# Thealexbarney/VGAudio

Hardware: AMD Instinct MI355X
Metric: Msamples/s encoded (GC-ADPCM, 4096 ch) at 1/2/4/8 GPUs; % HBM roofline (higher is better)
Workload: dtype int32; 1 GPU; BASELINE configs[1]: 4096 mono channels x 48 kHz x 60 s GC-ADPCM coefficient search + encode per GPU; parallelism=units sharded x1, channels_per_gpu=4096, samples_per_channel=2880000, bit_exact_channels_checked=0

## Files before the change

include/vgaudio_hip_testing.h:

```cpp
#ifndef VGAUDIO_HIP_TESTING_H
#define VGAUDIO_HIP_TESTING_H

#ifdef __cplusplus
extern "C" {
#endif

int vga_testing_force_open_seams_this_thread(int mode);

int vga_testing_gc_encoder_layout_this_thread(int channels_per_wave);
int vga_testing_gc_coefs_variant_this_thread(int variant);
int vga_testing_gc_encoder_segments_this_thread(int segments);
int vga_testing_gc_encoder_persistent_this_thread(int mode);

int vga_testing_gc_plan_pieces(int cus, int groups, int frames, long long group_frames, int ragged, int *out5);
int vga_testing_gc_plan_pieces_n(int cus, int groups, int frames, long long group_frames, int ragged, int coarse, int *out10);

int vga_testing_gc_encode_stats(unsigned long long *out8, int reset);
int vga_testing_gc_encode_stats_n(unsigned long long *out, int n, int reset);

int vga_testing_gc_seam_handover_this_thread(int on);
int vga_testing_gc_schedule_this_thread(int big_rounds, const int *tail_counts, const int *tail_frames, int min_tail_frames);
int vga_testing_gc_slow_order_host(const short *coefs, int nch, int *order);
int vga_testing_gc_slow_order_device(const void *d_coefs, int nch, int *order);
int vga_testing_gc_prologue_device(const void *d_coefs, int nch, int zero_ints, int *order_flags, int *bad_words);

void vga_testing_host_pipeline_this_thread(int feeders, int drainers, int chunk_units, int slot_bytes);

void vga_testing_host_pipeline_tail_this_thread(int tail_units);

int vga_testing_plan_buckets(const int *group, const int *length, int n, int max_units, long long max_volume, int longest_first,
                             int *order_out, int *chunk_begin_out, int *chunk_length_out, int *chunk_group_out, int max_chunks);
void vga_testing_buckets_order_this_thread(int order);
void vga_testing_host_transfer_this_thread(int mode);
void vga_testing_host_transfer_piece_bytes_this_thread(int bytes);
void vga_testing_host_compute_lanes_this_thread(int lanes);

enum {
    VGA_TESTING_STEP_CHUNK_COMPUTE = 1,
    VGA_TESTING_STEP_TRANSFER = 2,
    VGA_TESTING_STEP_HCA_STREAM_FRAMES = 3
};
void vga_testing_fail_step_this_thread(int kind, int nth);

int vga_testing_last_pipeline_stats(double *out, int n);

int vga_testing_hca_frames_per_group_this_thread(int frames);

int vga_testing_hca_device_info(const void *hca_info, void *out, int out_bytes);

int vga_testing_hca_decode_classes(const void *infos, int nstreams, int *class_out);
int vga_testing_hca_decode_v_stats(long long *out, int n);
int vga_testing_hca_ragged_stats(const void *ragged, long long *out, int n);

int vga_testing_adx_read_general_this_thread(int on);

int vga_testing_adx_last_path_this_thread(int *encode, int *decode);
int vga_testing_adx_ragged_stats(const void *ragged, long long *out, int n);

int vga_testing_poison_allocations(int byte);

#ifdef __cplusplus
}
#endif
// ... 2 lines not shown
```

vgaudio_amd/_lib.py:

```python
import ctypes as C
import importlib.util
import os

_HERE = os.path.dirname(os.path.abspath(__file__))
SO_PATH = os.environ.get("VGAUDIO_HIP_LIBRARY") or os.path.join(_HERE, "libvgaudio_hip.so")

VGA_OK = 0
VGA_ERR_ARGUMENT = -1
VGA_ERR_OUT_OF_RANGE = -2
VGA_ERR_INVALID_DATA = -3
VGA_ERR_INVALID_OP = -4
VGA_ERR_DEVICE = -5

VGA_TESTING_STEP_CHUNK_COMPUTE = 1
VGA_TESTING_STEP_TRANSFER = 2
VGA_TESTING_STEP_HCA_STREAM_FRAMES = 3


class VgaError(RuntimeError):
    code = None


class ArgumentError(VgaError, ValueError):
    code = VGA_ERR_ARGUMENT
# ... 80 lines not shown
    "vga_gcadpcm_encode_with_coefs_batch_v": (ci, [i16pp, C.POINTER(ci), ci, i16p, i16p, i16p, u8pp]),
    "vga_gcadpcm_decode_batch_v": (ci, [u8pp, i16p, C.POINTER(ci), ci, i16p, i16p, i16pp]),
    "vga_gcadpcm_ragged_create": (ci, [C.POINTER(ci), ci, C.POINTER(vp)]),
    "vga_gcadpcm_ragged_destroy": (None, [vp]),
    "vga_gcadpcm_ragged_channels": (ci, [vp]),
    "vga_gcadpcm_ragged_pcm_samples": (i64, [vp]),
    "vga_gcadpcm_ragged_adpcm_bytes": (i64, [vp]),
    "vga_gcadpcm_ragged_coefs_workspace_bytes": (C.c_size_t, [vp]),
    "vga_gcadpcm_ragged_offsets": (ci, [vp, C.POINTER(i64), C.POINTER(i64)]),
    "vga_gcadpcm_coefs_device_v": (ci, [vp, vp, vp, vp, C.c_size_t, vp]),
    "vga_gcadpcm_encode_device_v": (ci, [vp, vp, vp, vp, vp, vp, vp]),
    "vga_gcadpcm_decode_device_v": (ci, [vp, vp, vp, vp, vp, vp, vp, vp]),
    "encode": (None, [i16p, u8p, C.POINTER(ADPCMINFO), C.c_uint32]),
    "decode": (None, [u8p, i16p, C.POINTER(ADPCMINFO), C.c_uint32]),
    "correlateCoefs": (None, [i16p, C.c_uint32, i16p]),
    "encodeFrame": (None, [i16p, u8p, i16p, C.c_uint8]),
    "vga_gcadpcm_coefs_workspace_bytes": (C.c_size_t, [ci, ci]),
    "vga_gcadpcm_coefs_device": (ci, [vp, i64, ci, ci, vp, vp, C.c_size_t, vp]),
    "vga_gcadpcm_encode_device": (ci, [vp, i64, ci, ci, vp, vp, vp, vp, i64, vp]),
    "vga_gcadpcm_decode_device": (ci, [vp, i64, vp, ci, ci, vp, vp, vp, i64, vp, vp]),
    "vga_synth_pcm16_device": (ci, [vp, i64, ci, ci, ci, vp, vp]),
    "vga_adx_file_layout_for": (ci, [vp, ci, vp]),
    "vga_adx_write": (ci, [u8pp, ci, i16p, ci, vp, u8p]),
    "vga_adx_write_device": (ci, [vp, i64, ci, vp, ci, vp, vp, vp]),
    "vga_hca_file_size": (ci, [vp]),
    "vga_hca_file_header": (ci, [vp, C.c_char_p, C.c_float, ci, ci, u8p]),
    "vga_hca_write": (ci, [vp, u8p, C.c_char_p, C.c_float, ci, ci, u8p]),
    "vga_hca_write_device": (ci, [vp, vp, i64, ci, C.c_char_p, C.c_float, ci, ci, vp, i64, vp]),
    "vga_wave_parse": (ci, [u8p, i64, vp]),
    "vga_wave_read_pcm16": (ci, [u8p, i64, vp, i16pp]),
    "vga_wave_deinterleave_pcm16_device": (ci, [vp, ci, ci, vp, i64, vp]),
    "vga_wave_file_size": (i64, [vp, ci]),
    "vga_wave_write_pcm16": (ci, [i16pp, ci, vp, u8p]),
    "vga_wave_write_pcm16_device": (ci, [vp, i64, ci, vp, vp, vp]),
    "vga_adx_key_from_code": (ci, [C.c_uint64, vp]),
    "vga_adx_key_from_string": (ci, [C.c_char_p, vp]),
    "vga_adx_key_code": (C.c_uint64, [vp]),
    "vga_adx_crypt": (ci, [u8pp, ci, ci, vp, ci, ci]),
    "vga_adx_crypt_device": (ci, [vp, i64, ci, ci, vp, ci, ci, vp]),
    "vga_adx_find_key_device": (ci, [vp, i64, ci, ci, ci, ci, vp, ci, C.POINTER(ci), vp]),
    "vga_hca_key_tables": (ci, [ci, C.c_uint64, u8p, u8p]),
    "vga_hca_crypt": (ci, [u8p, ci, ci, u8p]),
    "vga_hca_find_key": (ci, [vp, u8p, ci, u8p, ci, vp]),
    "vga_hca_find_key_device": (ci, [vp, vp, ci, u8p, ci, vp, vp]),
    "vga_hca_byte_position_counts_device": (ci, [vp, i64, ci, ci, ci, ci, vp, vp]),
    "vga_adx_guess_default_candidates": (ci, [ci, vp, vp, vp, vp]),
    "vga_adx_guess_keys": (ci, [vp, ci, ci, ci, vp, ci, vp, ci, vp, ci, vp]),
    "vga_hca_crypt_device": (ci, [vp, i64, ci, ci, ci, u8p, vp]),
    "vga_release_cached_memory": (None, []),
    "vga_testing_force_open_seams_this_thread": (ci, [ci]),
    "vga_testing_host_pipeline_this_thread": (None, [ci, ci, ci, ci]),
    "vga_testing_gc_encoder_layout_this_thread": (ci, [ci]),
    "vga_testing_gc_coefs_variant_this_thread": (ci, [ci]),
    "vga_testing_gc_encoder_segments_this_thread": (ci, [ci]),
    "vga_testing_gc_encoder_persistent_this_thread": (ci, [ci]),
    "vga_testing_gc_seam_handover_this_thread": (ci, [ci]),
    "vga_testing_gc_schedule_this_thread": (ci, [ci, C.POINTER(ci), C.POINTER(ci), ci]),
    "vga_testing_gc_slow_order_host": (ci, [vp, ci, vp]),
    "vga_testing_gc_slow_order_device": (ci, [vp, ci, vp]),
    "vga_testing_gc_prologue_device": (ci, [vp, ci, ci, vp, vp]),
    "vga_testing_gc_encode_stats_n": (ci, [C.POINTER(C.c_ulonglong), ci, ci]),
    "vga_testing_last_pipeline_stats": (ci, [vp, ci]),
    "vga_testing_host_pipeline_tail_this_thread": (None, [ci]),
    "vga_testing_buckets_order_this_thread": (None, [ci]),
    "vga_testing_host_transfer_this_thread": (None, [ci]),
    "vga_testing_host_transfer_piece_bytes_this_thread": (None, [ci]),
    "vga_testing_host_compute_lanes_this_thread": (None, [ci]),
    "vga_testing_fail_step_this_thread": (None, [ci, ci]),
    "vga_testing_poison_allocations": (ci, [ci]),
    "vga_testing_plan_buckets": (ci, [C.POINTER(ci), C.POINTER(ci), ci, ci, C.c_longlong, ci, C.POINTER(ci), C.POINTER(ci), C.POINTER(ci),
                                 C.POINTER(ci), ci]),
    "vga_testing_hca_device_info": (ci, [vp, vp, ci]),
    "vga_testing_hca_decode_classes": (ci, [vp, ci, C.POINTER(ci)]),
    "vga_testing_hca_decode_v_stats": (ci, [C.POINTER(C.c_longlong), ci]),
    "vga_testing_hca_ragged_stats": (ci, [vp, C.POINTER(C.c_longlong), ci]),
    "vga_hca_ragged_layout_for": (ci, [vp, ci, C.POINTER(i64), C.POINTER(i64), vp]),
    "vga_hca_ragged_create": (ci, [vp, ci, C.POINTER(vp)]),
    "vga_hca_ragged_destroy": (None, [vp]),
    "vga_hca_ragged_streams": (ci, [vp]),
    "vga_hca_ragged_totals_of": (ci, [vp, vp]),
    "vga_hca_ragged_offsets": (ci, [vp, C.POINTER(i64), C.POINTER(i64)]),
    "vga_testing_adx_ragged_stats": (ci, [vp, C.POINTER(C.c_longlong), ci]),
    "vga_adx_ragged_layout_for": (ci, [vp, C.POINTER(ci), ci, C.POINTER(i64), C.POINTER(i64), vp]),
    "vga_adx_ragged_create": (ci, [vp, C.POINTER(ci), ci, C.POINTER(vp)]),
    "vga_adx_ragged_destroy": (None, [vp]),
    "vga_adx_ragged_channels": (ci, [vp]),
    "vga_adx_ragged_totals_of": (ci, [vp, vp]),
    "vga_adx_ragged_offsets": (ci, [vp, C.POINTER(i64), C.POINTER(i64)]),
    "vga_adx_encode_device_v": (ci, [vp, vp, vp, vp, vp, C.c_size_t, vp]),
    "vga_adx_decode_device_v": (ci, [vp, vp, vp, vp, C.c_size_t, vp, vp]),
    "vga_gc_files_layout_for": (ci, [vp, ci, vp, C.POINTER(ci), C.POINTER(i64), C.POINTER(i64), vp]),
    "vga_gc_files_create": (ci, [vp, ci, vp, C.POINTER(vp)]),
    "vga_gc_files_create_from_dsp": (ci, [C.POINTER(vp), ci, C.POINTER(i64), C.POINTER(vp)]),
    "vga_gc_files_destroy": (None, [vp]),
    "vga_gc_files_totals_of": (ci, [vp, vp]),
    "vga_gc_files_offsets": (ci, [vp, C.POINTER(ci), C.POINTER(i64), C.POINTER(i64)]),
    "vga_gc_files_ragged": (vp, [vp]),
    "vga_gcadpcm_build_channels_device_v": (ci, [vp, vp, vp, vp, vp, vp, vp, vp, C.c_size_t, vp]),
    "vga_dsp_write_device_v": (ci, [vp, vp, vp, vp, vp, vp, vp, vp]),
    "vga_dsp_read_device_v": (ci, [vp, vp, vp, vp, vp, vp, vp, vp]),
    "vga_gc_aligned_layout_for": (ci, [vp, ci, C.POINTER(ci), C.POINTER(i64), vp]),
    "vga_gc_aligned_create": (ci, [vp, ci, C.POINTER(vp)]),
    "vga_gc_aligned_destroy": (None, [vp]),
    "vga_gc_aligned_totals_of": (ci, [vp, vp]),
    "vga_gc_aligned_offsets": (ci, [vp, C.POINTER(ci), C.POINTER(i64)]),
    "vga_gc_aligned_ragged_in": (vp, [vp]),
# ... 564 lines not shown
```

vgaudio_amd/csrc/gcadpcm_kernels.hip:

```cpp
#include "common.hpp"
#include "gcadpcm_kernels.hpp"

#include <algorithm>
#include <cstdlib>
#include <type_traits>

namespace vga {
namespace gc {

struct Record {
    double r1, r2;
    bool valid;
};

__device__ __forceinline__ double get3(const double (&v)[3], int i) { return i == 0 ? v[0] : (i == 1 ? v[1] : v[2]); }
__device__ __forceinline__ void set3(double (&v)[3], int i, double val)
{
    if (i == 0) v[0] = val; else if (i == 1) v[1] = val; else v[2] = val;
}

struct FrameSums {
    double vec[3];
    double m11, m12, m22;
};

__device__ __forceinline__ FrameSums frame_sums(const int (&x)[16])
{
    FrameSums f;
#pragma unroll
    for (int i = 0; i <= 2; i++) {
        long long s = 0;
#pragma unroll
        for (int t = 0; t < 14; t++) s -= (long long)(x[2 + t - i] * x[2 + t]);
        f.vec[i] = (double)s;
    }
    long long s11 = 0, s12 = 0, s22 = 0;
#pragma unroll
    for (int z = 0; z < 14; z++) {
        s11 += (long long)(x[2 + z - 1] * x[2 + z - 1]);
        s12 += (long long)(x[2 + z - 1] * x[2 + z - 2]);
        s22 += (long long)(x[2 + z - 2] * x[2 + z - 2]);
    }
    f.m11 = (double)s11; f.m12 = (double)s12; f.m22 = (double)s22;
    return f;
}

typedef short short2v __attribute__((ext_vector_type(2)));
__device__ __forceinline__ int dot2_less1(uint32_t a, uint32_t b)
{
    return __builtin_amdgcn_sdot2(__builtin_bit_cast(short2v, a), __builtin_bit_cast(short2v, b), -1, false);
}
__device__ __forceinline__ FrameSums frame_sums_packed(const uint32_t (&w)[8])
{
    double s0 = 7.0, s1 = 7.0, s2 = 7.0;
#pragma unroll
    for (int i = 0; i < 7; i++) {
        s0 += (double)dot2_less1(w[i + 1], w[i + 1]);
        s1 += (double)dot2_less1(w[i], __builtin_amdgcn_alignbit(w[i + 1], w[i], 16));
        s2 += (double)dot2_less1(w[i], w[i + 1]);
    }
    const int x0 = (int)(int16_t)(w[0] & 0xFFFF), x1 = (int)w[0] >> 16;
    const int x14 = (int)(int16_t)(w[7] & 0xFFFF), x15 = (int)w[7] >> 16;
    FrameSums f;
    f.vec[0] = 0.0 - s0;
    f.vec[1] = 0.0 - ((s1 - (double)(x0 * x1)) + (double)(x14 * x15));
    f.vec[2] = 0.0 - s2;
    f.m12 = s1;
    f.m11 = (s0 + (double)(x1 * x1)) - (double)(x15 * x15);
    f.m22 = (f.m11 + (double)(x0 * x0)) - (double)(x14 * x14);
    return f;
}

__device__ __forceinline__ Record frame_record(const FrameSums &fs)
{
    Record rec;
    rec.valid = false;
    rec.r1 = rec.r2 = 0.0;

    double vec[3] = {fs.vec[0], fs.vec[1], fs.vec[2]};
    if (!(fabs(vec[0]) > 10.0)) return rec;

    double m11 = fs.m11, m12 = fs.m12, m21 = fs.m12, m22 = fs.m22;

    int idx1, idx2;
    {
        const double eps = 4.9406564584124654e-324;
        double val = fmax(fabs(m11), fabs(m12));
        if (val < eps) return rec;
        double rc1 = 1.0 / val;
        val = fmax(fabs(m21), fabs(m22));
        if (val < eps) return rec;
        double rc2 = 1.0 / val;

        int max_index = 0;
        double tmp;
        val = 0.0;
        tmp = fabs(m11) * rc1;
        if (tmp >= val) { val = tmp; max_index = 1; }
        tmp = fabs(m21) * rc2;
        if (tmp >= val) { val = tmp; max_index = 2; }
        if (max_index == 2) {
            double t;
            t = m21; m21 = m11; m11 = t;
            t = m22; m22 = m12; m12 = t;
            rc2 = rc1;
        }
        idx1 = max_index;
        tmp = 1.0 / m11;
        m21 *= tmp;
        val = 0.0;
        tmp = m22;
        tmp -= m21 * m12;
        m22 = tmp;
        tmp = fabs(tmp) * rc2;
        if (tmp >= val) { val = tmp; max_index = 2; }
        if (max_index == 1) {
            double t;
            t = m11; m11 = m21; m21 = t;
            t = m12; m12 = m22; m22 = t;
            rc1 = rc2;
        }
        idx2 = max_index;

        double mn = 1.0e10, mx = 0.0;
        tmp = fabs(m11);
        if (tmp < mn) mn = tmp;
        if (tmp > mx) mx = tmp;
        tmp = fabs(m22);
        if (tmp < mn) mn = tmp;
        if (tmp > mx) mx = tmp;
        if (mn / mx < 1.0e-10) return rec;
    }

    {
        double tmp;
        int xx = 0;
        tmp = get3(vec, idx1);
        set3(vec, idx1, vec[1]);
        if (xx != 0) {  }
        else if (tmp != 0.0) xx = 1;
        vec[1] = tmp;
        tmp = get3(vec, idx2);
        set3(vec, idx2, vec[2]);
        if (xx != 0) {
            if (xx == 1) tmp -= vec[1] * m21;
        } else if (tmp != 0.0) xx = 2;
        vec[2] = tmp;

        tmp = vec[2];
        vec[2] = tmp / m22;
        tmp = vec[1];
        tmp -= vec[2] * m12;
        vec[1] = tmp / m11;
        vec[0] = 1.0;
    }

    {
        const double v2 = vec[2];
        const double tmp = 1.0 - (v2 * v2);
        if (tmp == 0.0) return rec;
        const double v0 = (vec[0] - (v2 * v2)) / tmp;
        const double v1 = (vec[1] - (vec[1] * v2)) / tmp;
        vec[0] = v0;
        vec[1] = v1;
        if (fabs(v1) > 1.0) return rec;
    }

#pragma unroll
    for (int z = 1; z <= 2; z++) {
        if (vec[z] >= 1.0) vec[z] = 0.9999999999;
        else if (vec[z] <= -1.0) vec[z] = -0.9999999999;
    }
    rec.r1 = (vec[2] * vec[1]) + vec[1];
    rec.r2 = vec[2];
    rec.valid = true;
    return rec;
}

__device__ __forceinline__ void matrix_filter(double r1, double r2, double &d1, double &d2)
{
    const double m21 = -r1;
    const double m22 = -r2;
    const double val = 1.0 - (m22 * m22);
    const double m11 = ((m22 * m21) + m21) / val;
    d1 = 0.0 + m11 * 1.0;
    d2 = (0.0 + m21 * d1) + m22 * 1.0;
}

__device__ __forceinline__ void finish_record(double (&in_r)[3], double (&out_r)[3])
{
#pragma unroll
    for (int z = 1; z <= 2; z++) {
        if (in_r[z] >= 1.0) in_r[z] = 0.9999999999;
        else if (in_r[z] <= -1.0) in_r[z] = -0.9999999999;
    }
    out_r[0] = 1.0;
    out_r[1] = (in_r[2] * in_r[1]) + in_r[1];
    out_r[2] = in_r[2];
}

__device__ void merge_finish_record(const double (&src)[3], double (&dst)[3])
{
    double tmp[3] = {0.0, 0.0, 0.0};
    double val = src[0];
    dst[0] = 1.0;
    {
        double v2 = 0.0;
        if (val > 0.0) dst[1] = -(v2 + src[1]) / val;
        else dst[1] = 0.0;
        tmp[1] = dst[1];
        val *= 1.0 - (dst[1] * dst[1]);
    }
    {
        double v2 = 0.0;
        v2 += dst[1] * src[1];
        if (val > 0.0) dst[2] = -(v2 + src[2]) / val;
        else dst[2] = 0.0;
        tmp[2] = dst[2];
        dst[1] += dst[2] * dst[1];
        val *= 1.0 - (dst[2] * dst[2]);
    }
    finish_record(tmp, dst);
}


__device__ __forceinline__ void load_frame16(const int16_t *src, int f, int length, int (&x)[16])
{
    const int base = f * 14 - 2;
    if (f > 0 && base + 16 <= length) {
        const uint32_t *p32 = reinterpret_cast<const uint32_t *>(src + base);
#pragma unroll
        for (int i = 0; i < 8; i++) {
            const uint32_t w = p32[i];
            x[2 * i] = (int)(int16_t)(w & 0xFFFF);
            x[2 * i + 1] = (int)w >> 16;
        }
    } else {
#pragma unroll
        for (int i = 0; i < 16; i++) {
// ... 104 lines not shown
    __shared__ double s_vb[8][3];
    __shared__ double s_cw[8][3];
    __shared__ double s_sum[8][3];
    __shared__ int s_cnt[8];

    const int ch = rg.order ? rg.order[blockIdx.x] : (int)blockIdx.x;
    if (rg.order) length = rg.length[ch];
    const int lane = threadIdx.x;
    const int16_t *src = pcm + (rg.order ? rg.pcm_off[ch] : (int64_t)ch * pcm_pitch);
    const int frames = (length + 13) / 14;
    const int rec_pitch = (int)coef_record_pitch(frames);
    double2 *rec = records + (rg.order ? rg.rec_off[ch] : (int64_t)ch * rec_pitch);
    const int my_bucket = lane >> 1;
    const int my_comp = lane & 1;
    uint32_t wave_slot = 0;
    if (VGA_COEFS_PRIO == 1) asm volatile("s_getreg_b32 %0, hwreg(HW_REG_HW_ID, 0, 4)" : "=s"(wave_slot));
    if (VGA_COEFS_PRIO == 3) __builtin_amdgcn_s_setprio(3);
    const int64_t ragged_job = rg.order ? (int64_t)((rg.max_length + 13) / 14) * 7 : 0;
    auto ragged_priority = [&](int passes_left) __attribute__((always_inline)) {
        const int64_t q = 4 * (int64_t)frames * passes_left / (ragged_job > 0 ? ragged_job : 1);
        set_priority((uint32_t)(q > 3 ? 3 : q));
    };
    if (VGA_COEFS_PRIO == 3 && rg.order) ragged_priority(7);

    auto zero_fill = [&](int par) {
        reinterpret_cast<double2 *>(p0(par, 0))[lane] = make_double2(0.0, 0.0);
        reinterpret_cast<double2 *>(p0(par, 1))[lane] = make_double2(0.0, 0.0);
    };
    auto zero_fill2 = [&](int) {
        double2 *z = reinterpret_cast<double2 *>(ll(0));
#pragma unroll
        for (int q = 0; q < COEF_SLOTS / 64; q++) z[q * 64 + lane] = make_double2(0.0, 0.0);
    };

#ifdef VGA_DEBUG_TIMESTAMPS
    if (lane == 0) g_vga_coef_ts[3 * (blockIdx.x & 16383)] = wall_clock64();
#endif
    double acc = 0.0;
    int cnt = 0;
    int par = 0;
    const int f_hi = (length - 14) / 14;
    const bool have_interior = f_hi >= 1;
    uint32_t wr[COEF_PF_PCM][8];
    auto prefetch = [&](int f, uint32_t (&w)[8]) {
        const int fp = min(max(f, 1), max(f_hi, 1));
        const uint32_t *p32 = reinterpret_cast<const uint32_t *>(src + (int64_t)fp * 14 - 2);
#pragma unroll
        for (int i = 0; i < 8; i++) w[i] = p32[i];
    };
    if (have_interior) {
#pragma unroll
        for (int q = 0; q < COEF_PF_PCM; q++) prefetch(lane + 64 * q, wr[q]);
    }
    auto record_chunk = [&](int base, const uint32_t (&wc)[8]) __attribute__((always_inline)) {
        const int f = base + lane;
        bool valid = false;
        double d1 = 0.0, d2 = 0.0;
        if (f < frames) {
            FrameSums fs;
            if (have_interior && f >= 1 && f <= f_hi) {
                fs = frame_sums_packed(wc);
            } else {
                int x[16];
                load_frame16(src, f, length, x);
                fs = frame_sums(x);
            }
            Record r;
            if (VGA_COEFS_ABLATE & 8) { r.valid = fs.vec[0] != 0.0; r.r1 = fs.m11 * 1e-12; r.r2 = fs.m12 * 1e-12; }
            else r = frame_record(fs);
            valid = r.valid;
            if (valid) { if (VGA_COEFS_ABLATE & 8) { d1 = r.r1; d2 = r.r2; } else matrix_filter(r.r1, r.r2, d1, d2); }
            rec[record_position(f)] = valid ? make_double2(d1, d2) : make_double2(__builtin_nan(""), 0.0);
        }
        const uint64_t mask = __ballot(valid);
        const int n = __popcll(mask);
        zero_fill(par);
        if (valid) {
            const int slot = lane_rank(mask);
            p0(par, 0)[slot] = d1;
            p0(par, 1)[slot] = d2;
        }
        wave_lds_sync();
        if (lane < 2 && !(VGA_COEFS_ABLATE & 16)) acc = ordered_sum(acc, p0(par, lane), n, n);
        rotate_priority(wave_slot);
        cnt += n;
        par ^= 1;
    };
    for (int base = 0; base < frames; base += 64 * COEF_PF_PCM) {
#pragma unroll
        for (int q = 0; q < COEF_PF_PCM; q++) {
            if (base + 64 * q < frames) {
                uint32_t wc[8];
#pragma unroll
                for (int i = 0; i < 8; i++) wc[i] = wr[q][i];
                if (have_interior) prefetch(base + 64 * (q + COEF_PF_PCM) + lane, wr[q]);
                record_chunk(base + 64 * q, wc);
            }
        }
    }
#ifdef VGA_DEBUG_TIMESTAMPS
    if (lane == 0) g_vga_coef_ts[3 * (blockIdx.x & 16383) + 1] = wall_clock64();
#endif
    __syncthreads();
    if (lane < 2) s_sum[0][1 + lane] = acc;
    __syncthreads();
    if (lane == 0) {
        double vec1[3];
        vec1[0] = 1.0;
        vec1[1] = s_sum[0][1];
        vec1[2] = s_sum[0][2];
        vec1[1] /= cnt;
        vec1[2] /= cnt;
        double vb[3];
        merge_finish_record(vec1, vb);
        s_vb[0][0] = vb[0]; s_vb[0][1] = vb[1]; s_vb[0][2] = vb[2];
    }
    __syncthreads();

    auto lloyd_iterations = [&](auto exp_c) {
        constexpr int EXP = decltype(exp_c)::value;
        for (int iter = 0; iter < 2; iter++) {
            if (VGA_COEFS_PRIO == 3) {
                if (rg.order) ragged_priority((EXP == 2 ? 6 : (EXP == 4 ? 4 : 2)) - iter);
                else set_priority(EXP == 2 ? 2 : (EXP == 4 ? 1 : 0));
            }
            if (lane < EXP) {
                const double a = s_vb[lane][0], b = s_vb[lane][1], c = s_vb[lane][2];
                s_cw[lane][0] = (a * a) + (b * b) + (c * c);
                s_cw[lane][1] = (a * b) + (b * c);
                s_cw[lane][2] = a * c;
            }
            __syncthreads();
            double cw1[EXP], cw2[EXP], cw3[EXP];
#pragma unroll
            for (int i = 0; i < EXP; i++) {
                cw1[i] = s_cw[i][0];
                cw2[i] = s_cw[i][1];
                cw3[i] = s_cw[i][2];
            }

            acc = 0.0;
            cnt = 0;
            auto classify = [&](int f, const double2 r, bool &valid, int &idx) __attribute__((always_inline)) {
                valid = false;
                idx = 0;
                if (f < frames && r.x == r.x) {
                    valid = true;
                    const double val_x2 = 2.0 * r.x, bterm_x2 = 2.0 * r.y;
                    double value = 1.0e30;
                    if (VGA_COEFS_ABLATE & 2) idx = (int)(__double_as_longlong(val_x2) >> 40) & (EXP - 1);
                    else {
#pragma unroll
                    for (int i = 0; i < EXP; i++) {
                        const double t = cw1[i] + (val_x2 * cw2[i]) + (bterm_x2 * cw3[i]);
                        idx = t < value ? i : idx;
                        asm("v_min_f64 %0, %1, %2" : "=v"(value) : "v"(value), "v"(t));
                    }
                    }
                }
            };
            using Fields = std::conditional_t<(EXP > 4), uint64_t, uint32_t>;
            auto field = [](Fields w, int i) __attribute__((always_inline)) { return (int)((w >> (8 * i)) & 0xFF); };
            auto lloyd_chunks = [&](int base, const double2 (&r)[COEF_K]) __attribute__((always_inline)) {
                bool v[COEF_K];
                int ix[COEF_K];
                Fields before[COEF_K], mine = 0;
#pragma unroll
                for (int k = 0; k < COEF_K; k++) {
                    classify(base + COEF_K * lane + k, r[k], v[k], ix[k]);
                    if (VGA_COEFS_ABLATE & 4) ix[k] = 0;
                    before[k] = mine;
                    mine += v[k] ? (Fields)1 << (8 * ix[k]) : (Fields)0;
                }
                const Fields lower = scan_fields(mine);
                const Fields lower63 = last_lane(lower), mine63 = last_lane(mine);
                int start = 0, max_n = 0;
                Fields starts = 0;
#pragma unroll
                for (int b = 0; b < EXP; b++) {
                    const int n = field(lower63, b) + field(mine63, b);
                    starts |= (Fields)(start >> 3) << (8 * b);
                    start += (n + 7) & ~7;
                    max_n = max(max_n, n);
                }
                zero_fill2(0);
#pragma unroll
                for (int k = 0; k < COEF_K; k++)
                    if (v[k]) {
                        const int slot = 8 * field(starts, ix[k]) + field(lower + before[k], ix[k]);
                        ll(0)[slot] = r[k].x;
                        ll(1)[slot] = r[k].y;
                    }
                wave_lds_sync();
                        if (lane < 2 * EXP && !(VGA_COEFS_ABLATE & 1)) {
                    const int my_n = field(lower63, my_bucket) + field(mine63, my_bucket);
                    acc = ordered_sum(acc, ll(my_comp) + 8 * field(starts, my_bucket), my_n, max_n);
                    cnt += my_n;
                }
                        rotate_priority(wave_slot);
            };
            double2 nxt[COEF_K];
#pragma unroll
            for (int k = 0; k < COEF_K; k++) nxt[k] = rec[lane + 64 * k];
            for (int base = 0; base < frames; base += 64 * COEF_K) {
                double2 cur[COEF_K];
#pragma unroll
                for (int k = 0; k < COEF_K; k++) {
                    cur[k] = nxt[k];
                    nxt[k] = rec[min(base + 64 * (COEF_K + k) + lane, rec_pitch - 1)];
                }
                lloyd_chunks(base, cur);
            }
            __syncthreads();
            if (lane < 2 * EXP) {
                s_sum[my_bucket][1 + my_comp] = acc;
                if (my_comp == 0) s_cnt[my_bucket] = cnt;
            }
            __syncthreads();
            if (lane < EXP) {
                double bl[3];
                const int n = s_cnt[lane];
                bl[0] = (double)n;
                bl[1] = s_sum[lane][1];
                bl[2] = s_sum[lane][2];
                if (n > 0) { bl[0] /= n; bl[1] /= n; bl[2] /= n; }
                double vb[3] = {s_vb[lane][0], s_vb[lane][1], s_vb[lane][2]};
                merge_finish_record(bl, vb);
                s_vb[lane][0] = vb[0]; s_vb[lane][1] = vb[1]; s_vb[lane][2] = vb[2];
            }
            __syncthreads();
        }
    };

    for (int w = 0; w < ((VGA_COEFS_ABLATE & 32) ? 0 : 3); w++) {
        const int half = 1 << w;
        if (lane < half) {
            s_vb[half + lane][0] = (0.01 * 0.0) + s_vb[lane][0];
            s_vb[half + lane][1] = (0.01 * -1.0) + s_vb[lane][1];
            s_vb[half + lane][2] = (0.01 * 0.0) + s_vb[lane][2];
        }
        __syncthreads();

        if (w == 0) lloyd_iterations(std::integral_constant<int, 2>{});
        else if (w == 1) lloyd_iterations(std::integral_constant<int, 4>{});
        else lloyd_iterations(std::integral_constant<int, 8>{});
    }

    if (lane < 16) {
        const int z = lane >> 1;
        const double d = -s_vb[z][1 + (lane & 1)] * 2048.0;
        int out;
        if (d > 0.0) out = (d > 32767.0) ? 32767 : (int)__builtin_rint(d);
        else out = (d < -32768.0) ? -32768 : ((d != d) ? 0 : (int)__builtin_rint(d));
        coefs_out[ch * 16 + lane] = (int16_t)out;
    }
#ifdef VGA_DEBUG_TIMESTAMPS
    if (lane == 0) g_vga_coef_ts[3 * (blockIdx.x & 16383) + 2] = wall_clock64();
#endif
}

constexpr int COEF_CW = 4;
constexpr int COEF_THREADS = (COEF_CW + 1) * 64;

template <bool SOLO>
__global__ __launch_bounds__(COEF_THREADS) __attribute__((amdgpu_waves_per_eu(5, 5))) void gc_coefs_kernel4(
    const int16_t *__restrict__ pcm, int64_t pcm_pitch, int nch, int length,
    double2 *__restrict__ records, int16_t *__restrict__ coefs_out, const Ragged rg)
{
    __shared__ __align__(64) double s_d[COEF_CW][2][2][128];
    __shared__ int s_meta[2][COEF_CW][8];
    __shared__ int s_maxn[2][COEF_CW];
    __shared__ double s_vb[COEF_CW][8][3];
    __shared__ double s_cw[COEF_CW][8][3];

    const int wave = threadIdx.x >> 6, lane = threadIdx.x & 63;
    const bool summer = wave == COEF_CW;
    const int ws = summer ? 0 : wave;
// ... 18 lines not shown
    double acc = 0.0;
    int cnt = 0;
    auto sum_chunk = [&](int par, int nb) {
        if (SOLO) {
#pragma unroll
            for (int w4 = 0; w4 < COEF_CW; w4++) {
                const int meta = s_meta[par][w4][sb];
                const int n = (sc == 0 && sb < nb) ? (meta & 0xFF) : 0;
                acc = ordered_sum(acc, &s_d[w4][par][sk][meta >> 8], n, s_maxn[par][w4]);
                cnt += n;
            }
        } else {
            const int meta = s_meta[par][sc][sb];
            const int trip = max(max(s_maxn[par][0], s_maxn[par][1]), max(s_maxn[par][2], s_maxn[par][3]));
            const int n = sb < nb ? (meta & 0xFF) : 0;
            acc = ordered_sum(acc, &s_d[sc][par][sk][meta >> 8], n, trip);
            cnt += n;
        }
    };

    const int f_hi = (length - 14) / 14;
    const bool have_interior = f_hi >= 1;
    uint32_t w[8];
    auto prefetch = [&](int f) {
        const int fp = min(max(f, 1), max(f_hi, 1));
        const uint32_t *p32 = reinterpret_cast<const uint32_t *>(src + (int64_t)fp * 14 - 2);
#pragma unroll
        for (int i = 0; i < 8; i++) w[i] = p32[i];
    };
    if (!summer && have_interior) prefetch(cfirst * 64 + lane);
    for (int rd = 0; rd < rounds; rd++) {
        const int par = rd & 1;
        const int c = rd * cstep + cfirst;
        if (!summer) {
            const int f = c * 64 + lane;
            bool valid = false;
            double d1 = 0.0, d2 = 0.0;
            uint32_t wc[8];
#pragma unroll
            for (int i = 0; i < 8; i++) wc[i] = w[i];
            if (have_interior) prefetch(f + 64 * cstep);
            if (f < frames) {
                FrameSums fs;
                if (have_interior && f >= 1 && f <= f_hi) {
                    fs = frame_sums_packed(wc);
                } else {
                    int x[16];
                    load_frame16(src, f, length, x);
                    fs = frame_sums(x);
                }
                const Record r = frame_record(fs);
                valid = r.valid && live;
                if (valid) matrix_filter(r.r1, r.r2, d1, d2);
                if (live) rec[f] = valid ? make_double2(d1, d2) : make_double2(__builtin_nan(""), 0.0);
            }
            const uint64_t mask = __ballot(valid);
            const int n = __popcll(mask);
            zero_fill(par);
            if (valid) {
                const int slot = lane_rank(mask);
                s_d[ws][par][0][slot] = d1;
                s_d[ws][par][1][slot] = d2;
            }
            if (lane < 8) s_meta[par][ws][lane] = lane == 0 ? n : 0;
            if (lane == 8) s_maxn[par][ws] = n;
        } else if (rd > 0) {
            sum_chunk(par ^ 1, 1);
        }
        lds_barrier();
    }
    if (summer) {
        if (rounds > 0) sum_chunk((rounds - 1) & 1, 1);
        const double other = __shfl_xor(acc, 1);
        if (sb == 0 && sk == 0) {
            double vec1[3];
            vec1[0] = 1.0;
            vec1[1] = acc;
            vec1[2] = other;
            vec1[1] /= cnt;
            vec1[2] /= cnt;
            double vb[3];
            merge_finish_record(vec1, vb);
            s_vb[sc][0][0] = vb[0]; s_vb[sc][0][1] = vb[1]; s_vb[sc][0][2] = vb[2];
        }
    }
    lds_barrier();

    auto lloyd_iterations = [&](auto exp_c) {
        constexpr int EXP = decltype(exp_c)::value;
        for (int iter = 0; iter < 2; iter++) {
            if (!summer && lane < EXP && (!SOLO || wave == 0)) {
                const double a = s_vb[cs][lane][0], b = s_vb[cs][lane][1], c3 = s_vb[cs][lane][2];
                s_cw[cs][lane][0] = (a * a) + (b * b) + (c3 * c3);
                s_cw[cs][lane][1] = (a * b) + (b * c3);
                s_cw[cs][lane][2] = a * c3;
            }
            lds_barrier();
            double cw1[EXP], cw2[EXP], cw3[EXP];
#pragma unroll
            for (int i = 0; i < EXP; i++) {
                cw1[i] = s_cw[cs][i][0];
                cw2[i] = s_cw[cs][i][1];
                cw3[i] = s_cw[cs][i][2];
            }
            acc = 0.0;
            cnt = 0;
            double2 r_next = make_double2(0.0, 0.0);
            if (!summer && frames > 0) r_next = rec[min(cfirst * 64 + lane, frames - 1)];
            for (int rd = 0; rd < rounds; rd++) {
                const int par = rd & 1;
                const int c = rd * cstep + cfirst;
                if (!summer) {
                    const int f = c * 64 + lane;
                    bool valid = false;
                    int idx = 0;
                    double d1 = 0.0, d2 = 0.0;
                    const double2 r = r_next;
                    r_next = rec[min(f + 64 * cstep, frames - 1)];
                    if (live && f < frames && r.x == r.x) {
                        valid = true;
                        const double val_x2 = 2.0 * r.x, bterm_x2 = 2.0 * r.y;
                        double value = 1.0e30;
#pragma unroll
                        for (int i = 0; i < EXP; i++) {
                            const double t = cw1[i] + (val_x2 * cw2[i]) + (bterm_x2 * cw3[i]);
                            idx = t < value ? i : idx;
                            asm("v_min_f64 %0, %1, %2" : "=v"(value) : "v"(value), "v"(t));
                        }
                        d1 = r.x;
                        d2 = r.y;
                    }
                    int slot = 0, my_meta = 0, start = 0, max_n = 0;
#pragma unroll
                    for (int b = 0; b < EXP; b++) {
                        const bool mine = valid && idx == b;
                        const uint64_t m = __ballot(mine);
                        const int n_b = __popcll(m);
                        if (mine) slot = start + lane_rank(m);
                        if (lane == b) my_meta = (start << 8) | n_b;
                        start += (n_b + 7) & ~7;
                        max_n = max(max_n, n_b);
                    }
                    zero_fill(par);
                    if (valid) {
                        s_d[ws][par][0][slot] = d1;
                        s_d[ws][par][1][slot] = d2;
                    }
                    if (lane < 8) s_meta[par][ws][lane] = my_meta;
                    if (lane == 8) s_maxn[par][ws] = max_n;
                } else if (rd > 0) {
                    sum_chunk(par ^ 1, EXP);
                }
                lds_barrier();
            }
            if (summer) {
                if (rounds > 0) sum_chunk((rounds - 1) & 1, EXP);
                const double other = __shfl_xor(acc, 1);
                if (sb < EXP && sk == 0) {
                    double bl[3];
                    const int n = cnt;
                    bl[0] = (double)n;
                    bl[1] = acc;
                    bl[2] = other;
                    if (n > 0) { bl[0] /= n; bl[1] /= n; bl[2] /= n; }
                    double vb[3] = {s_vb[sc][sb][0], s_vb[sc][sb][1], s_vb[sc][sb][2]};
                    merge_finish_record(bl, vb);
                    s_vb[sc][sb][0] = vb[0]; s_vb[sc][sb][1] = vb[1]; s_vb[sc][sb][2] = vb[2];
                }
            }
            lds_barrier();
        }
    };

    for (int wsplit = 0; wsplit < 3; wsplit++) {
        const int half = 1 << wsplit;
        if (!summer && lane < half && (!SOLO || wave == 0)) {
            s_vb[cs][half + lane][0] = (0.01 * 0.0) + s_vb[cs][lane][0];
            s_vb[cs][half + lane][1] = (0.01 * -1.0) + s_vb[cs][lane][1];
            s_vb[cs][half + lane][2] = (0.01 * 0.0) + s_vb[cs][lane][2];
        }
        lds_barrier();
        if (wsplit == 0) lloyd_iterations(std::integral_constant<int, 2>{});
        else if (wsplit == 1) lloyd_iterations(std::integral_constant<int, 4>{});
        else lloyd_iterations(std::integral_constant<int, 8>{});
    }

    if (live && lane < 16 && (!SOLO || wave == 0)) {
        const int z = lane >> 1;
        const double d = -s_vb[cs][z][1 + (lane & 1)] * 2048.0;
        int out;
        if (d > 0.0) out = (d > 32767.0) ? 32767 : (int)__builtin_rint(d);
        else out = (d < -32768.0) ? -32768 : ((d != d) ? 0 : (int)__builtin_rint(d));
        coefs_out[ch * 16 + lane] = (int16_t)out;
    }
}

__device__ __forceinline__ uint64_t splitmix64(uint64_t x)
{
    x += 0x9E3779B97F4A7C15ull;
    uint64_t z = x;
    z = (z ^ (z >> 30)) * 0xBF58476D1CE4E5B9ull;
    z = (z ^ (z >> 27)) * 0x94D049BB133111EBull;
    return z ^ (z >> 31);
}
__device__ __forceinline__ long long tri(uint32_t phase)
{
    const long long q = (long long)(phase >> 15);
    return q < 65536 ? q - 32768 : 98303 - q;
}

__global__ __launch_bounds__(256) void synth_kernel(int16_t *__restrict__ pcm, int64_t pitch, int nch, int length,
                                                    int first_channel, const uint32_t *__restrict__ params)
{
    const int k = blockIdx.y;
    const int c = first_channel + k;
    const uint32_t f_inc = params[4 * k + 0], phi = params[4 * k + 1], amp = params[4 * k + 2], lfo = params[4 * k + 3];
// ... 26 lines not shown
    if (nch <= 0 || usable == 0) return 0;
    const double scale = 256.0 / (double)(cus > 0 ? cus : 256);
    const double longest = (double)((lengths_longest_first[0] + 13) / 14), total = (double)total_frames;
    const double five_waves = std::max(longest * 4.8e-5, total / 1.27e7 * scale);
    const double one_wave = std::max(longest * 7.1e-5, total / 2.16e7 * scale);
    return five_waves < one_wave ? usable : 0;
}

int launch_coefs(const int16_t *d_pcm, int64_t pcm_pitch, int nch, int length, int16_t *d_coefs,
                 void *d_workspace, hipStream_t stream, const Ragged *rg)
{
    if (nch <= 0) return VGA_OK;
    if (rg) {
        const int solo = coefs_kernel_variant() == 1 ? 0 : (coefs_kernel_variant() == 3 ? rg->solo_usable : rg->solo_channels);
        Ragged rest = *rg;
        rest.order += solo;
        if (solo > 0)
            hipLaunchKernelGGL(gc_coefs_kernel4<true>, dim3(solo), dim3(COEF_THREADS), 0, stream, d_pcm, (int64_t)0, solo, 0,
                               reinterpret_cast<double2 *>(d_workspace), d_coefs, *rg);
        if (solo < nch)
            hipLaunchKernelGGL(gc_coefs_kernel, dim3(nch - solo), dim3(64), 0, stream, d_pcm, (int64_t)0, nch, 0,
                               reinterpret_cast<double2 *>(d_workspace), d_coefs, rest);
        VGA_HIP_TRY(hipGetLastError());
        return VGA_OK;
    }
    const int variant = coefs_kernel_variant();
    const bool solo = variant == 3 || (variant == 0 && nch <= device_cu_count() * SOLO_WORKGROUPS_PER_CU);
    const bool per_channel = variant == 1 || (variant == 0 && !solo);
    if (per_channel)
        hipLaunchKernelGGL(gc_coefs_kernel, dim3(nch), dim3(64), 0, stream, d_pcm, pcm_pitch, nch, length,
                           reinterpret_cast<double2 *>(d_workspace), d_coefs, Ragged{});
    else if (solo)
        hipLaunchKernelGGL(gc_coefs_kernel4<true>, dim3(nch), dim3(COEF_THREADS), 0, stream, d_pcm, pcm_pitch, nch, length,
                           reinterpret_cast<double2 *>(d_workspace), d_coefs, Ragged{});
    else
        hipLaunchKernelGGL(gc_coefs_kernel4<false>, dim3((nch + COEF_CW - 1) / COEF_CW), dim3(COEF_THREADS), 0, stream, d_pcm, pcm_pitch,
                           nch, length, reinterpret_cast<double2 *>(d_workspace), d_coefs, Ragged{});
    VGA_HIP_TRY(hipGetLastError());
    return VGA_OK;
}

int launch_synth(int16_t *d_pcm, int64_t pitch, int nch, int length, int first_channel, const uint32_t *d_params,
                 hipStream_t stream)
{
    if (nch <= 0 || length <= 0) return VGA_OK;
    int gx = (int)((length + 255) / 256);
    if (gx > 1024) gx = 1024;
    hipLaunchKernelGGL(synth_kernel, dim3(gx, nch), dim3(256), 0, stream, d_pcm, pitch, nch, length, first_channel,
                       d_params);
    VGA_HIP_TRY(hipGetLastError());
    return VGA_OK;
}

}
}
```

Baseline: 94300 Msamples/s.

## Slim GC-ADPCM coefficient search arithmetic with reciprocal division and simplified LU pivoting

Moves the frame-record and codeword helpers into a shared host/device header and reduces their arithmetic. It drops the second pivot step, replaces two divisions with a refined hardware reciprocal plus FMA correction, and checks the ratio with multiplies instead of a division, falling back to exact division when any lane is near the boundary. It also stores records pre-doubled so the codeword search skips the scaling and halves the sums later, uses a direct LDS write when every lane is valid, and adds a coalesced record position when 64 divides evenly by the chunk factor. These changes risk bit-exactness of the coefficients, which the reciprocal fallback paths and a new quotient test kernel are meant to guard.

New measurement: 94890 Msamples/s (median of 6 runs). Within noise of the previous version (+0.6%).

```diff
diff --git a/include/vgaudio_hip_testing.h b/include/vgaudio_hip_testing.h
--- a/include/vgaudio_hip_testing.h
+++ b/include/vgaudio_hip_testing.h
@@ -9,6 +9,7 @@
 
 int vga_testing_gc_encoder_layout_this_thread(int channels_per_wave);
 int vga_testing_gc_coefs_variant_this_thread(int variant);
+int vga_testing_gc_coefs_quotient(const double *num, const double *den, int n, double *out, unsigned char *fast);
 int vga_testing_gc_encoder_segments_this_thread(int segments);
 int vga_testing_gc_encoder_persistent_this_thread(int mode);
 
diff --git a/vgaudio_amd/_lib.py b/vgaudio_amd/_lib.py
--- a/vgaudio_amd/_lib.py
+++ b/vgaudio_amd/_lib.py
@@ -156,6 +156,7 @@
     "vga_testing_host_pipeline_this_thread": (None, [ci, ci, ci, ci]),
     "vga_testing_gc_encoder_layout_this_thread": (ci, [ci]),
     "vga_testing_gc_coefs_variant_this_thread": (ci, [ci]),
+    "vga_testing_gc_coefs_quotient": (ci, [vp, vp, ci, vp, vp]),
     "vga_testing_gc_encoder_segments_this_thread": (ci, [ci]),
     "vga_testing_gc_encoder_persistent_this_thread": (ci, [ci]),
     "vga_testing_gc_seam_handover_this_thread": (ci, [ci]),
diff --git a/vgaudio_amd/csrc/gc_coefs_core.hpp b/vgaudio_amd/csrc/gc_coefs_core.hpp
--- /dev/null
+++ b/vgaudio_amd/csrc/gc_coefs_core.hpp
@@ -0,0 +1,209 @@
+#pragma once
+#include <cmath>
+#include <cstdint>
+
+#if defined(__HIPCC__)
+#define VGA_HD __host__ __device__ __forceinline__
+#else
+#define VGA_HD inline
+#endif
+#if defined(__HIP_DEVICE_COMPILE__)
+#define VGA_COEFS_ANY(p) (__any(p) != 0)
+#else
+#define VGA_COEFS_ANY(p) (p)
+#endif
+
+#ifndef VGA_COEFS_LEAN
+#define VGA_COEFS_LEAN 0xFF
+#endif
+
+namespace vga {
+namespace gc {
+
+struct Reciprocal {
+    double d, y;
+};
+VGA_HD bool division_range(double x) { return fabs(x) >= 0x1p-200 && fabs(x) <= 0x1p200; }
+VGA_HD Reciprocal refined_reciprocal(double d)
+{
+    Reciprocal r;
+    r.d = d;
+#if defined(__HIP_DEVICE_COMPILE__)
+    double y = __builtin_amdgcn_rcp(d);
+    double e = __builtin_fma(-d, y, 1.0);
+    y = __builtin_fma(y, e, y);
+    e = __builtin_fma(-d, y, 1.0);
+    r.y = __builtin_fma(y, e, y);
+#else
+    r.y = 0.0;
+#endif
+    return r;
+}
+VGA_HD double quotient(double n, const Reciprocal &r)
+{
+#if defined(__HIP_DEVICE_COMPILE__)
+    const double q = n * r.y;
+    const double e = __builtin_fma(-r.d, q, n);
+    return __builtin_fma(e, r.y, q);
+#else
+    return n / r.d;
+#endif
+}
+
+struct Record {
+    double r1, r2;
+    bool valid;
+};
+
+struct FrameSums {
+    double vec[3];
+    double m11, m12, m22;
+};
+
+VGA_HD double get3(const double (&v)[3], int i) { return i == 0 ? v[0] : (i == 1 ? v[1] : v[2]); }
+VGA_HD void set3(double (&v)[3], int i, double val)
+{
+    if (i == 0) v[0] = val; else if (i == 1) v[1] = val; else v[2] = val;
+}
+
+VGA_HD bool lu_ratio_below_1e10(double mn, double mx)
+{
+    if (!(VGA_COEFS_LEAN & 1)) return mn / mx < 1.0e-10;
+    const double lo = 0.5e-10 * mx, hi = 2.0e-10 * mx;
+    const bool below = mn <= lo;
+    const bool between = !below && !(mn >= hi);
+    if (VGA_COEFS_ANY(between)) return mn / mx < 1.0e-10;
+    return below;
+}
+
+VGA_HD Record frame_record(const FrameSums &fs)
+{
+    Record rec;
+    rec.valid = false;
+    rec.r1 = rec.r2 = 0.0;
+
+    double vec[3] = {fs.vec[0], fs.vec[1], fs.vec[2]};
+    if (!(fabs(vec[0]) > 10.0)) return rec;
+
+    double m11 = fs.m11, m12 = fs.m12, m21 = fs.m12, m22 = fs.m22;
+
+    int idx1;
+    Reciprocal pivot;
+    pivot.d = pivot.y = 0.0;
+    {
+        const double eps = 4.9406564584124654e-324;
+        double val = fmax(fabs(m11), fabs(m12));
+        if (val < eps) return rec;
+        double rc1 = 1.0 / val;
+        val = fmax(fabs(m21), fabs(m22));
+        if (val < eps) return rec;
+        double rc2 = 1.0 / val;
+
+        int max_index = 0;
+        double tmp;
+        val = 0.0;
+        tmp = fabs(m11) * rc1;
+        if (tmp >= val) { val = tmp; max_index = 1; }
+        tmp = fabs(m21) * rc2;
+        if (tmp >= val) { val = tmp; max_index = 2; }
+        if (max_index == 2) {
+            double t;
+            t = m21; m21 = m11; m11 = t;
+            t = m22; m22 = m12; m12 = t;
+        }
+        idx1 = max_index;
+        if (VGA_COEFS_LEAN & 2) { pivot = refined_reciprocal(m11); tmp = quotient(1.0, pivot); }
+        else tmp = 1.0 / m11;
+        m21 *= tmp;
+        tmp = m22;
+        tmp -= m21 * m12;
+        m22 = tmp;
+
+        double mn = 1.0e10, mx = 0.0;
+        tmp = fabs(m11);
+        if (tmp < mn) mn = tmp;
+        if (tmp > mx) mx = tmp;
+        tmp = fabs(m22);
+        if (tmp < mn) mn = tmp;
+        if (tmp > mx) mx = tmp;
+        if (lu_ratio_below_1e10(mn, mx)) return rec;
+    }
+
+    {
+        double tmp;
+        int xx = 0;
+        tmp = get3(vec, idx1);
+        set3(vec, idx1, vec[1]);
+        if (xx != 0) {  }
+        else if (tmp != 0.0) xx = 1;
+        vec[1] = tmp;
+        tmp = vec[2];
+        if (xx != 0) {
+            if (xx == 1) tmp -= vec[1] * m21;
+        } else if (tmp != 0.0) xx = 2;
+        vec[2] = tmp;
+
+        tmp = vec[2];
+        vec[2] = tmp / m22;
+        tmp = vec[1];
+        tmp -= vec[2] * m12;
+        if (!(VGA_COEFS_LEAN & 2) || VGA_COEFS_ANY(!division_range(tmp))) vec[1] = tmp / m11;
+        else vec[1] = quotient(tmp, pivot);
+        vec[0] = 1.0;
+    }
+
+    {
+        const double v2 = vec[2];
+        const double tmp = 1.0 - (v2 * v2);
+        if (tmp == 0.0) return rec;
+        const double v0 = (vec[0] - (v2 * v2)) / tmp;
+        const double v1 = (vec[1] - (vec[1] * v2)) / tmp;
+        vec[0] = v0;
+        vec[1] = v1;
+        if (fabs(v1) > 1.0) return rec;
+    }
+
+    for (int z = 1; z <= 2; z++) {
+        if (vec[z] >= 1.0) vec[z] = 0.9999999999;
+        else if (vec[z] <= -1.0) vec[z] = -0.9999999999;
+    }
+    rec.r1 = (vec[2] * vec[1]) + vec[1];
+    rec.r2 = vec[2];
+    rec.valid = true;
+    return rec;
+}
+
+VGA_HD void matrix_filter(double r1, double r2, double &d1, double &d2)
+{
+    const double m21 = -r1;
+    const double m22 = -r2;
+    const double val = 1.0 - (m22 * m22);
+    const double m11 = ((m22 * m21) + m21) / val;
+    d1 = 0.0 + m11 * 1.0;
+    d2 = (0.0 + m21 * d1) + m22 * 1.0;
+}
+
+VGA_HD double doubled_for_record(double d) { return (VGA_COEFS_LEAN & 32) ? 2.0 * d : d; }
+VGA_HD double halve_sum(double s2) { return (VGA_COEFS_LEAN & 32) ? 0.5 * s2 : s2; }
+
+template <int EXP>
+VGA_HD int nearest_codeword(double x2, double y2, const double (&cw1)[EXP], const double (&cw2)[EXP], const double (&cw3)[EXP])
+{
+    if (!(VGA_COEFS_LEAN & 32)) { x2 *= 2.0; y2 *= 2.0; }
+    double value = 1.0e30;
+    int idx = 0;
+#pragma unroll
+    for (int i = 0; i < EXP; i++) {
+        const double t = cw1[i] + (x2 * cw2[i]) + (y2 * cw3[i]);
+        idx = t < value ? i : idx;
+#if defined(__HIP_DEVICE_COMPILE__)
+        asm("v_min_f64 %0, %1, %2" : "=v"(value) : "v"(value), "v"(t));
+#else
+        value = t < value ? t : value;
+#endif
+    }
+    return idx;
+}
+
+}
+}
diff --git a/vgaudio_amd/csrc/gcadpcm_kernels.hip b/vgaudio_amd/csrc/gcadpcm_kernels.hip
--- a/vgaudio_amd/csrc/gcadpcm_kernels.hip
+++ b/vgaudio_amd/csrc/gcadpcm_kernels.hip
@@ -1,5 +1,6 @@
 #include "common.hpp"
 #include "gcadpcm_kernels.hpp"
+#include "gc_coefs_core.hpp"
 
 #include <algorithm>
 #include <cstdlib>
@@ -7,22 +8,6 @@
 
 namespace vga {
 namespace gc {
-
-struct Record {
-    double r1, r2;
-    bool valid;
-};
-
-__device__ __forceinline__ double get3(const double (&v)[3], int i) { return i == 0 ? v[0] : (i == 1 ? v[1] : v[2]); }
-__device__ __forceinline__ void set3(double (&v)[3], int i, double val)
-{
-    if (i == 0) v[0] = val; else if (i == 1) v[1] = val; else v[2] = val;
-}
-
-struct FrameSums {
-    double vec[3];
-    double m11, m12, m22;
-};
 
 __device__ __forceinline__ FrameSums frame_sums(const int (&x)[16])
 {
@@ -69,122 +54,6 @@
     f.m11 = (s0 + (double)(x1 * x1)) - (double)(x15 * x15);
     f.m22 = (f.m11 + (double)(x0 * x0)) - (double)(x14 * x14);
     return f;
-}
-
-__device__ __forceinline__ Record frame_record(const FrameSums &fs)
-{
-    Record rec;
-    rec.valid = false;
-    rec.r1 = rec.r2 = 0.0;
-
-    double vec[3] = {fs.vec[0], fs.vec[1], fs.vec[2]};
-    if (!(fabs(vec[0]) > 10.0)) return rec;
-
-    double m11 = fs.m11, m12 = fs.m12, m21 = fs.m12, m22 = fs.m22;
-
-    int idx1, idx2;
-    {
-        const double eps = 4.9406564584124654e-324;
-        double val = fmax(fabs(m11), fabs(m12));
-        if (val < eps) return rec;
-        double rc1 = 1.0 / val;
-        val = fmax(fabs(m21), fabs(m22));
-        if (val < eps) return rec;
-        double rc2 = 1.0 / val;
-
-        int max_index = 0;
-        double tmp;
-        val = 0.0;
-        tmp = fabs(m11) * rc1;
-        if (tmp >= val) { val = tmp; max_index = 1; }
-        tmp = fabs(m21) * rc2;
-        if (tmp >= val) { val = tmp; max_index = 2; }
-        if (max_index == 2) {
-            double t;
-            t = m21; m21 = m11; m11 = t;
-            t = m22; m22 = m12; m12 = t;
-            rc2 = rc1;
-        }
-        idx1 = max_index;
-        tmp = 1.0 / m11;
-        m21 *= tmp;
-        val = 0.0;
-        tmp = m22;
-        tmp -= m21 * m12;
-        m22 = tmp;
-        tmp = fabs(tmp) * rc2;
-        if (tmp >= val) { val = tmp; max_index = 2; }
-        if (max_index == 1) {
-            double t;
-            t = m11; m11 = m21; m21 = t;
-            t = m12; m12 = m22; m22 = t;
-            rc1 = rc2;
-        }
-        idx2 = max_index;
-
-        double mn = 1.0e10, mx = 0.0;
-        tmp = fabs(m11);
-        if (tmp < mn) mn = tmp;
-        if (tmp > mx) mx = tmp;
-        tmp = fabs(m22);
-        if (tmp < mn) mn = tmp;
-        if (tmp > mx) mx = tmp;
-        if (mn / mx < 1.0e-10) return rec;
-    }
-
-    {
-        double tmp;
-        int xx = 0;
-        tmp = get3(vec, idx1);
-        set3(vec, idx1, vec[1]);
-        if (xx != 0) {  }
-        else if (tmp != 0.0) xx = 1;
-        vec[1] = tmp;
-        tmp = get3(vec, idx2);
-        set3(vec, idx2, vec[2]);
-        if (xx != 0) {
-            if (xx == 1) tmp -= vec[1] * m21;
-        } else if (tmp != 0.0) xx = 2;
-        vec[2] = tmp;
-
-        tmp = vec[2];
-        vec[2] = tmp / m22;
-        tmp = vec[1];
-        tmp -= vec[2] * m12;
-        vec[1] = tmp / m11;
-        vec[0] = 1.0;
-    }
-
-    {
-        const double v2 = vec[2];
-        const double tmp = 1.0 - (v2 * v2);
-        if (tmp == 0.0) return rec;
-        const double v0 = (vec[0] - (v2 * v2)) / tmp;
-        const double v1 = (vec[1] - (vec[1] * v2)) / tmp;
-        vec[0] = v0;
-        vec[1] = v1;
-        if (fabs(v1) > 1.0) return rec;
-    }
-
-#pragma unroll
-    for (int z = 1; z <= 2; z++) {
-        if (vec[z] >= 1.0) vec[z] = 0.9999999999;
-        else if (vec[z] <= -1.0) vec[z] = -0.9999999999;
-    }
-    rec.r1 = (vec[2] * vec[1]) + vec[1];
-    rec.r2 = vec[2];
-    rec.valid = true;
-    return rec;
-}
-
-__device__ __forceinline__ void matrix_filter(double r1, double r2, double &d1, double &d2)
-{
-    const double m21 = -r1;
-    const double m22 = -r2;
-    const double val = 1.0 - (m22 * m22);
-    const double m11 = ((m22 * m21) + m21) / val;
-    d1 = 0.0 + m11 * 1.0;
-    d2 = (0.0 + m21 * d1) + m22 * 1.0;
 }
 
 __device__ __forceinline__ void finish_record(double (&in_r)[3], double (&out_r)[3])
@@ -395,6 +264,7 @@
 #pragma unroll
         for (int q = 0; q < COEF_PF_PCM; q++) prefetch(lane + 64 * q, wr[q]);
     }
+    const int rec_lane = 64 * (lane % COEF_K) + lane / COEF_K;
     auto record_chunk = [&](int base, const uint32_t (&wc)[8]) __attribute__((always_inline)) {
         const int f = base + lane;
         bool valid = false;
@@ -413,15 +283,21 @@
             else r = frame_record(fs);
             valid = r.valid;
             if (valid) { if (VGA_COEFS_ABLATE & 8) { d1 = r.r1; d2 = r.r2; } else matrix_filter(r.r1, r.r2, d1, d2); }
-            rec[record_position(f)] = valid ? make_double2(d1, d2) : make_double2(__builtin_nan(""), 0.0);
+            const int pos = (64 % COEF_K == 0) ? (base - base % (64 * COEF_K)) + (base % (64 * COEF_K)) / COEF_K + rec_lane : record_position(f);
+            rec[pos] = valid ? make_double2(doubled_for_record(d1), doubled_for_record(d2)) : make_double2(__builtin_nan(""), 0.0);
         }
         const uint64_t mask = __ballot(valid);
         const int n = __popcll(mask);
-        zero_fill(par);
-        if (valid) {
-            const int slot = lane_rank(mask);
-            p0(par, 0)[slot] = d1;
-            p0(par, 1)[slot] = d2;
+        if ((VGA_COEFS_LEAN & 16) && mask == ~0ull) {
+            p0(par, 0)[lane] = d1;
+            p0(par, 1)[lane] = d2;
+        } else {
+            zero_fill(par);
+            if (valid) {
+                const int slot = lane_rank(mask);
+                p0(par, 0)[slot] = d1;
+                p0(par, 1)[slot] = d2;
+            }
         }
         wave_lds_sync();
         if (lane < 2 && !(VGA_COEFS_ABLATE & 16)) acc = ordered_sum(acc, p0(par, lane), n, n);
@@ -489,17 +365,8 @@
                 idx = 0;
                 if (f < frames && r.x == r.x) {
                     valid = true;
-                    const double val_x2 = 2.0 * r.x, bterm_x2 = 2.0 * r.y;
-                    double value = 1.0e30;
-                    if (VGA_COEFS_ABLATE & 2) idx = (int)(__double_as_longlong(val_x2) >> 40) & (EXP - 1);
-                    else {
-#pragma unroll
-                    for (int i = 0; i < EXP; i++) {
-                        const double t = cw1[i] + (val_x2 * cw2[i]) + (bterm_x2 * cw3[i]);
-                        idx = t < value ? i : idx;
-                        asm("v_min_f64 %0, %1, %2" : "=v"(value) : "v"(value), "v"(t));
-                    }
-                    }
+                    if (VGA_COEFS_ABLATE & 2) idx = (int)(__double_as_longlong(r.x) >> 40) & (EXP - 1);
+                    else idx = nearest_codeword<EXP>(r.x, r.y, cw1, cw2, cw3);
                 }
             };
             using Fields = std::conditional_t<(EXP > 4), uint64_t, uint32_t>;
@@ -564,8 +431,8 @@
                 double bl[3];
                 const int n = s_cnt[lane];
                 bl[0] = (double)n;
-                bl[1] = s_sum[lane][1];
-                bl[2] = s_sum[lane][2];
+                bl[1] = halve_sum(s_sum[lane][1]);
+                bl[2] = halve_sum(s_sum[lane][2]);
                 if (n > 0) { bl[0] /= n; bl[1] /= n; bl[2] /= n; }
                 double vb[3] = {s_vb[lane][0], s_vb[lane][1], s_vb[lane][2]};
                 merge_finish_record(bl, vb);
@@ -690,7 +557,7 @@
                 const Record r = frame_record(fs);
                 valid = r.valid && live;
                 if (valid) matrix_filter(r.r1, r.r2, d1, d2);
-                if (live) rec[f] = valid ? make_double2(d1, d2) : make_double2(__builtin_nan(""), 0.0);
+                if (live) rec[f] = valid ? make_double2(doubled_for_record(d1), doubled_for_record(d2)) : make_double2(__builtin_nan(""), 0.0);
             }
             const uint64_t mask = __ballot(valid);
             const int n = __popcll(mask);
@@ -757,14 +624,7 @@
                     r_next = rec[min(f + 64 * cstep, frames - 1)];
                     if (live && f < frames && r.x == r.x) {
                         valid = true;
-                        const double val_x2 = 2.0 * r.x, bterm_x2 = 2.0 * r.y;
-                        double value = 1.0e30;
-#pragma unroll
-                        for (int i = 0; i < EXP; i++) {
-                            const double t = cw1[i] + (val_x2 * cw2[i]) + (bterm_x2 * cw3[i]);
-                            idx = t < value ? i : idx;
-                            asm("v_min_f64 %0, %1, %2" : "=v"(value) : "v"(value), "v"(t));
-                        }
+                        idx = nearest_codeword<EXP>(r.x, r.y, cw1, cw2, cw3);
                         d1 = r.x;
                         d2 = r.y;
                     }
@@ -798,8 +658,8 @@
                     double bl[3];
                     const int n = cnt;
                     bl[0] = (double)n;
-                    bl[1] = acc;
-                    bl[2] = other;
+                    bl[1] = halve_sum(acc);
+                    bl[2] = halve_sum(other);
                     if (n > 0) { bl[0] /= n; bl[1] /= n; bl[2] /= n; }
                     double vb[3] = {s_vb[sc][sb][0], s_vb[sc][sb][1], s_vb[sc][sb][2]};
                     merge_finish_record(bl, vb);
@@ -932,5 +792,40 @@
     return VGA_OK;
 }
 
-}
-}
+__global__ __launch_bounds__(64) void gc_quotient_test_kernel(const double *__restrict__ num, const double *__restrict__ den, int n,
+                                                              double *__restrict__ out, unsigned char *__restrict__ fast)
+{
+    const int i = (int)blockIdx.x * 64 + (int)threadIdx.x;
+    if (i >= n) return;
+    const double a = num[i], d = den[i];
+    double q;
+    unsigned char f = 0;
+    if (VGA_COEFS_ANY(!(division_range(a) && division_range(d)))) q = a / d;
+    else {
+        q = quotient(a, refined_reciprocal(d));
+        f = 1;
+    }
+    out[i] = q;
+    fast[i] = f;
+}
+
+}
+}
+
+extern "C" int vga_testing_gc_coefs_quotient(const double *num, const double *den, int n, double *out, unsigned char *fast)
+{
+    if (!num || !den || !out || !fast || n <= 0) return -1;
+    const size_t bytes = (size_t)n * sizeof(double);
+    char *d = nullptr;
+    if (hipMalloc(&d, 3 * bytes + (size_t)n) != hipSuccess) return -1;
+    double *d_num = reinterpret_cast<double *>(d), *d_den = d_num + n, *d_out = d_den + n;
+    unsigned char *d_fast = reinterpret_cast<unsigned char *>(d_out + n);
+    bool ok = hipMemcpy(d_num, num, bytes, hipMemcpyHostToDevice) == hipSuccess && hipMemcpy(d_den, den, bytes, hipMemcpyHostToDevice) == hipSuccess;
+    if (ok) {
+        hipLaunchKernelGGL(vga::gc::gc_quotient_test_kernel, dim3((unsigned)((n + 63) / 64)), dim3(64), 0, (hipStream_t)0, d_num, d_den, n, d_out, d_fast);
+        ok = hipGetLastError() == hipSuccess && hipMemcpy(out, d_out, bytes, hipMemcpyDeviceToHost) == hipSuccess &&
+             hipMemcpy(fast, d_fast, (size_t)n, hipMemcpyDeviceToHost) == hipSuccess;
+    }
+    (void)hipFree(d);
+    return ok ? 0 : -1;
+}
```
